# seungjunlee96/lightning-generative-models

Measured on AMD Instinct MI355X. Metric: training images/sec (DDPM UNet 32x32, bs=128), higher is better.
Workload: dtype f32

## Files before the change

### lightning-generative-models_amd/csrc/linattn_fused.hip

```cpp
#include <type_traits>

#include "lgm_common.h"

int lgm_wgrad_reduce_launch(const float* ws, long slab, float* gw, long n_w, float* gb, long n_b, int splits, float beta,
                            hipStream_t s);

namespace {

constexpr int DH = 32;
constexpr int HEADS = 4;
constexpr int HID = HEADS * DH;
constexpr int C = 64;
constexpr int LD = 36;
constexpr int TP = 128;
constexpr int XLD = 80;
constexpr int WLD = 100;

struct FArgs {
  const float* qkv;  long pitch;
  const float* gout; long gout_pitch;
  const float* ctx; const float* gctx; const float* kmax; const float* ksum; const float* rvec;
  const float* xn;   long xn_pitch;
  const float* wt;
  float* gxn;        long gxn_pitch;
  float* slabs;
  int n, tiles, items, per;
  float scale;
};

__device__ __forceinline__ void load16(const float* p, float (&v)[16]) {
#pragma unroll
  for (int q = 0; q < 4; ++q) {
    const f32x4 t = *reinterpret_cast<const f32x4*>(p + 4 * q);
    v[4 * q] = t[0]; v[4 * q + 1] = t[1]; v[4 * q + 2] = t[2]; v[4 * q + 3] = t[3];
  }
}

__global__ __launch_bounds__(256, 1) void linattn_bwd_fused_kernel(const FArgs p) {
  extern __shared__ __align__(16) float sm[];
  float* Qs = sm;
  float* Ks = Qs + TP * LD;
  float* Vs = Ks + TP * LD;
  float* Gs = Vs + TP * LD;
  float* Cs = Gs + TP * LD;
  float* GCs = Cs + DH * LD;
  float* GCt = GCs + DH * LD;
  float* rr = GCt + DH * LD;
  float* Ws = rr + DH;
  float* Xs = Ws + C * WLD;
  const int tid = threadIdx.x;
  const int lane = tid & 63, wid = tid >> 6;
  const int lr = lane & 31, lh = lane >> 5;
  const int l16 = lane & 15, lq = lane >> 4;
  const int c4 = (tid & 7) * 4, prow = tid >> 3;
  const int srow = 32 * wid + (lane >> 1), spart = (lane & 1) * 16;
  const int it0 = blockIdx.x * p.per, it1 = min(p.items, it0 + p.per);
  if (it0 >= it1) return;

  int w_src[6], w_dst[6];
#pragma unroll
  for (int u = 0; u < 6; ++u) {
    const int e = tid + 256 * u;
    const int c = e / 24, rem = e - 24 * c;
    const int part = rem >> 3, j = rem & 7;
    w_src[u] = c * (3 * HID) + part * HID + 4 * j;
    w_dst[u] = c * WLD + part * DH + 4 * j;
  }

  f32x4 q4[4], k4[4], v4[4], g4[4], km4, ks4, cx4, gc4, w4[6];
  float rr1 = 0.f;
  auto issue = [&](int it, int h) {
    const int b = it / p.tiles, i0 = (it % p.tiles) * TP;
    const int rows = min(TP, p.n - i0);
    const long bh = (long)b * HEADS + h;
#pragma unroll
    for (int u = 0; u < 4; ++u) {
      const int r = prow + 32 * u;
      const long row = (long)b * p.n + i0 + (r < rows ? r : 0);
      const float* qp = p.qkv + row * p.pitch + h * DH + c4;
      q4[u] = *reinterpret_cast<const f32x4*>(qp);
      k4[u] = *reinterpret_cast<const f32x4*>(qp + HID);
      v4[u] = *reinterpret_cast<const f32x4*>(qp + 2 * HID);
      g4[u] = *reinterpret_cast<const f32x4*>(p.gout + row * p.gout_pitch + h * DH + c4);
    }
    km4 = *reinterpret_cast<const f32x4*>(p.kmax + bh * DH + c4);
    ks4 = *reinterpret_cast<const f32x4*>(p.ksum + bh * DH + c4);
    cx4 = *reinterpret_cast<const f32x4*>(p.ctx + bh * DH * DH + tid * 4);
    gc4 = *reinterpret_cast<const f32x4*>(p.gctx + bh * DH * DH + tid * 4);
    if (tid < DH) rr1 = p.rvec[bh * DH + tid];
#pragma unroll
    for (int u = 0; u < 6; ++u) w4[u] = *reinterpret_cast<const f32x4*>(p.wt + w_src[u] + h * DH);
  };

  f32x4 dacc[HEADS][6];
#pragma unroll
  for (int h = 0; h < HEADS; ++h)
#pragma unroll
    for (int t = 0; t < 6; ++t) dacc[h][t] = f32x4{0.f, 0.f, 0.f, 0.f};
  const f32x4 zero4 = {0.f, 0.f, 0.f, 0.f};

  issue(it0, 0);
  for (int it = it0; it < it1; ++it) {
    const int b = it / p.tiles, i0 = (it % p.tiles) * TP;
    const int rows = min(TP, p.n - i0);
    f32x16 acc[2];
#pragma unroll
    for (int a = 0; a < 2; ++a)
#pragma unroll
      for (int r = 0; r < 16; ++r) acc[a][r] = 0.f;
    {
#pragma unroll
      for (int u = 0; u < 4; ++u) {
        const int r = prow + 32 * u;
        const long row = (long)b * p.n + i0 + (r < rows ? r : 0);
#pragma unroll
        for (int hf = 0; hf < 2; ++hf) {
          f32x4 xv = *reinterpret_cast<const f32x4*>(p.xn + row * p.xn_pitch + hf * 32 + c4);
          if (r >= rows) xv = zero4;
          *reinterpret_cast<f32x4*>(Xs + r * XLD + hf * 32 + c4) = xv;
        }
      }
    }
    auto head = [&](auto hc) {
      constexpr int h = decltype(hc)::value;
#pragma unroll
      for (int u = 0; u < 4; ++u) {
        const int r = prow + 32 * u;
        const bool live = r < rows;
        f32x4 kv;
#pragma unroll
        for (int k = 0; k < 4; ++k) kv[k] = __expf(k4[u][k] - km4[k]) * (1.f / ks4[k]);
        *reinterpret_cast<f32x4*>(Qs + r * LD + c4) = live ? q4[u] : zero4;
        *reinterpret_cast<f32x4*>(Ks + r * LD + c4) = live ? kv : zero4;
        *reinterpret_cast<f32x4*>(Vs + r * LD + c4) = live ? v4[u] : zero4;
        *reinterpret_cast<f32x4*>(Gs + r * LD + c4) = live ? g4[u] : zero4;
      }
      {
        const int d = tid >> 3, e0 = (tid & 7) * 4;
        *reinterpret_cast<f32x4*>(Cs + d * LD + e0) = cx4;
        *reinterpret_cast<f32x4*>(GCs + d * LD + e0) = gc4;
#pragma unroll
        for (int k = 0; k < 4; ++k) GCt[(e0 + k) * LD + d] = gc4[k];
      }
      if (tid < DH) rr[tid] = rr1;
#pragma unroll
      for (int u = 0; u < 6; ++u) *reinterpret_cast<f32x4*>(Ws + w_dst[u]) = w4[u];
      __syncthreads();
      if (h + 1 < HEADS) issue(it, h + 1);
      else if (it + 1 < it1) issue(it + 1, 0);

      float sv[16];
      {
        load16(Qs + srow * LD + spart, sv);
        float mx = sv[0];
#pragma unroll
        for (int k = 1; k < 16; ++k) mx = fmaxf(mx, sv[k]);
        mx = fmaxf(mx, __shfl_xor(mx, 1, 64));
        float sum = 0.f;
#pragma unroll
        for (int k = 0; k < 16; ++k) {
          sv[k] = __expf(sv[k] - mx);
          sum += sv[k];
        }
        sum += __shfl_xor(sum, 1, 64);
        const float inv = 1.f / sum;
#pragma unroll
        for (int k = 0; k < 16; ++k) sv[k] *= inv;
      }
      f32x16 a1, a2, a3;
#pragma unroll
      for (int r = 0; r < 16; ++r) a1[r] = a2[r] = a3[r] = 0.f;
      {
        float ca[16], ga[16], ta[16], gb[16], vb[16], kb[16];
        load16(Cs + lr * LD + 16 * lh, ca);
        load16(GCs + lr * LD + 16 * lh, ga);
        load16(GCt + lr * LD + 16 * lh, ta);
        load16(Gs + (32 * wid + lr) * LD + 16 * lh, gb);
        load16(Vs + (32 * wid + lr) * LD + 16 * lh, vb);
        load16(Ks + (32 * wid + lr) * LD + 16 * lh, kb);
#pragma unroll
        for (int s = 0; s < 16; ++s) {
          a1 = __builtin_amdgcn_mfma_f32_32x32x2f32(ca[s], gb[s], a1, 0, 0, 0);
          a2 = __builtin_amdgcn_mfma_f32_32x32x2f32(ga[s], vb[s], a2, 0, 0, 0);
          a3 = __builtin_amdgcn_mfma_f32_32x32x2f32(ta[s], kb[s], a3, 0, 0, 0);
        }
      }
      lgm_wave_lds_sync();
      {
        float* gp = Gs + (32 * wid + lr) * LD + 4 * lh;
        float* vp = Vs + (32 * wid + lr) * LD + 4 * lh;
#pragma unroll
        for (int g = 0; g < 4; ++g) {
          *reinterpret_cast<f32x4*>(gp + 8 * g) = f32x4{a1[4 * g], a1[4 * g + 1], a1[4 * g + 2], a1[4 * g + 3]};
          *reinterpret_cast<f32x4*>(vp + 8 * g) = f32x4{a2[4 * g], a2[4 * g + 1], a2[4 * g + 2], a2[4 * g + 3]};
        }
      }
      lgm_wave_lds_sync();
      {
        float g1[16], t2[16], kk[16], rv[16], dot = 0.f;
        load16(Gs + srow * LD + spart, g1);
        load16(Vs + srow * LD + spart, t2);
        load16(Ks + srow * LD + spart, kk);
        load16(rr + spart, rv);
#pragma unroll
        for (int k = 0; k < 16; ++k) {
          g1[k] *= p.scale;
          dot += sv[k] * g1[k];
        }
        dot += __shfl_xor(dot, 1, 64);
#pragma unroll
        for (int q = 0; q < 4; ++q) {
          f32x4 oq, ok;
#pragma unroll
          for (int k = 0; k < 4; ++k) {
            oq[k] = sv[4 * q + k] * (g1[4 * q + k] - dot);
            ok[k] = kk[4 * q + k] * (t2[4 * q + k] - rv[4 * q + k]);
          }
          *reinterpret_cast<f32x4*>(Qs + srow * LD + spart + 4 * q) = oq;
          *reinterpret_cast<f32x4*>(Ks + srow * LD + spart + 4 * q) = ok;
        }
      }
      lgm_wave_lds_sync();
      {
        float* vp = Vs + (32 * wid + lr) * LD + 4 * lh;
#pragma unroll
        for (int g = 0; g < 4; ++g)
          *reinterpret_cast<f32x4*>(vp + 8 * g) = f32x4{a3[4 * g], a3[4 * g + 1], a3[4 * g + 2], a3[4 * g + 3]};
      }
      lgm_wave_lds_sync();
#pragma unroll
      for (int part = 0; part < 3; ++part) {
        float xb[16], w0[16], w1[16];
        load16((part == 0 ? Qs : part == 1 ? Ks : Vs) + (32 * wid + lr) * LD + 16 * lh, xb);
        load16(Ws + lr * WLD + part * DH + 16 * lh, w0);
        load16(Ws + (32 + lr) * WLD + part * DH + 16 * lh, w1);
#pragma unroll
        for (int s = 0; s < 16; ++s) {
          acc[0] = __builtin_amdgcn_mfma_f32_32x32x2f32(w0[s], xb[s], acc[0], 0, 0, 0);
          acc[1] = __builtin_amdgcn_mfma_f32_32x32x2f32(w1[s], xb[s], acc[1], 0, 0, 0);
        }
      }
      __syncthreads();
      {
        const float* xb = Xs + lq * XLD + 16 * wid + l16;
#pragma unroll 4
        for (int s = 0; s < TP / 4; ++s) {
          const float bv = xb[4 * s * XLD];
#pragma unroll
          for (int part = 0; part < 3; ++part) {
            const float* X = (part == 0 ? Qs : part == 1 ? Ks : Vs) + (4 * s + lq) * LD + l16;
            dacc[h][2 * part] = __builtin_amdgcn_mfma_f32_16x16x4f32(X[0], bv, dacc[h][2 * part], 0, 0, 0);
            dacc[h][2 * part + 1] = __builtin_amdgcn_mfma_f32_16x16x4f32(X[16], bv, dacc[h][2 * part + 1], 0, 0, 0);
          }
        }
        __syncthreads();
      }
    };
    head(std::integral_constant<int, 0>{});
    head(std::integral_constant<int, 1>{});
    head(std::integral_constant<int, 2>{});
    head(std::integral_constant<int, 3>{});
    if (32 * wid + lr < rows) {
      float* o = p.gxn + ((long)b * p.n + i0 + 32 * wid + lr) * p.gxn_pitch + 4 * lh;
#pragma unroll
      for (int a = 0; a < 2; ++a)
#pragma unroll
        for (int g = 0; g < 4; ++g)
          *reinterpret_cast<f32x4*>(o + 32 * a + 8 * g) = f32x4{acc[a][4 * g], acc[a][4 * g + 1], acc[a][4 * g + 2], acc[a][4 * g + 3]};
    }
  }
  {
    float* sl = p.slabs + (long)blockIdx.x * (3 * HID * C);
#pragma unroll
    for (int h = 0; h < HEADS; ++h)
#pragma unroll
      for (int t = 0; t < 6; ++t)
#pragma unroll
        for (int r = 0; r < 4; ++r) {
          const int wrow = (t >> 1) * HID + h * DH + (t & 1) * 16 + 4 * lq + r;
          sl[(long)wrow * C + 16 * wid + l16] = dacc[h][t][r];
        }
  }
}

constexpr size_t kSmem = ((size_t)4 * TP * LD + 3 * DH * LD + DH + C * WLD + TP * XLD) * sizeof(float);

int plan_blocks(int B, int n, int* tiles, int* items, int* per) {
  *tiles = lgm_cdiv(n, TP);
  *items = B * *tiles;
  const int nb = *items < 256 ? *items : 256;
  *per = lgm_cdiv(*items, nb);
  return lgm_cdiv(*items, *per);
}

}

extern "C" int64_t lgm_linattn_bwd_fused_supported(int heads, int dim_head, int Cin) {
  return heads == HEADS && dim_head == DH && Cin == C ? 1 : 0;
}

extern "C" int64_t lgm_linattn_bwd_fused_slabs(int B, int n, int Cin) {
  if (Cin != C) return 0;
  int tiles, items, per;
  const int blocks = plan_blocks(B, n, &tiles, &items, &per);
  return (int64_t)blocks * 3 * HID * C * (int64_t)sizeof(float);
}

int lgm_linattn_bwd_fused_launch(const float* qkv, long pitch, const float* gout, long gout_pitch, const float* ctx,
                                 const float* gctx, const float* kmax, const float* ksum, const float* rvec,
                                 const float* xn, long xn_pitch, const float* wt, int B, int n, float scale,
                                 float* gxn, long gxn_pitch, float* slabs, int* blocks_out, hipStream_t s) {
  FArgs a;
  a.qkv = qkv; a.pitch = pitch; a.gout = gout; a.gout_pitch = gout_pitch;
  a.ctx = ctx; a.gctx = gctx; a.kmax = kmax; a.ksum = ksum; a.rvec = rvec;
  a.xn = xn; a.xn_pitch = xn_pitch; a.wt = wt; a.gxn = gxn; a.gxn_pitch = gxn_pitch;
  a.slabs = slabs; a.n = n; a.scale = scale;
  const int blocks = plan_blocks(B, n, &a.tiles, &a.items, &a.per);
  *blocks_out = blocks;
  lgm_note_kernel(LGM_KNAME("linattn_bwd_fused_kernel"));
  static bool attr = false;
  if (!attr) {
    (void)hipFuncSetAttribute(reinterpret_cast<const void*>(linattn_bwd_fused_kernel),
                              hipFuncAttributeMaxDynamicSharedMemorySize, (int)kSmem);
    attr = true;
  }
  hipLaunchKernelGGL(linattn_bwd_fused_kernel, dim3(blocks), dim3(256), kSmem, s, a);
  LGM_LAUNCH_CHECK();
  return LGM_OK;
}

namespace {

constexpr int OTP = 128;
constexpr int ALD = 132;

struct OArgs {
  const float* qkv;  long pitch;
  const float* ctx;
  const float* wout; const float* bout; const float* g;
  const float* x;    long x_pitch;
  float* ao;         long ao_pitch;
  float* o2;         long o2_pitch;
  float* y;          long y_pitch;
  int n, tiles, items, per;
  float scale;
};

template <int NC>
__global__ __launch_bounds__(256, NC == 2 ? 3 : 1) void linattn_out_fused_kernel(const OArgs p) {
  constexpr int CO = 32 * NC;
  extern __shared__ __align__(16) float sm[];
  float* Ws = sm;
  float* Ct = Ws + CO * ALD;
  const int tid = threadIdx.x;
  const int lane = tid & 63, wid = tid >> 6;
  const int lr = lane & 31, lh = lane >> 5;
  const int it0 = blockIdx.x * p.per, it1 = min(p.items, it0 + p.per);
  if (it0 >= it1) return;
  const float sqrtc = sqrtf((float)CO);

  f32x4 qn[4];
  auto issue_q = [&](int it, int h) {
    const int b = it / p.tiles, i0 = (it % p.tiles) * OTP;
    const int pix = min(i0 + 32 * wid + lr, p.n - 1);
    const float* qp = p.qkv + ((long)b * p.n + pix) * p.pitch + h * DH + 16 * lh;
#pragma unroll
    for (int j = 0; j < 4; ++j) qn[j] = *reinterpret_cast<const f32x4*>(qp + 4 * j);
  };
  issue_q(it0, 0);
#pragma unroll
  for (int u = 0; u < NC * 4; ++u) {
    const int e = tid + 256 * u;
    const int c = e >> 5, k4 = (e & 31) * 4;
    *reinterpret_cast<f32x4*>(Ws + c * ALD + k4) = *reinterpret_cast<const f32x4*>(p.wout + (long)c * HID + k4);
  }
  int b_staged = -1;
  for (int it = it0; it < it1; ++it) {
    const int b = it / p.tiles, i0 = (it % p.tiles) * OTP;
    const int pix = i0 + 32 * wid + lr;
    const bool live = pix < p.n;
    const long row = (long)b * p.n + min(pix, p.n - 1);
    if (b != b_staged) {
      __syncthreads();
#pragma unroll
      for (int u = 0; u < 4; ++u) {
        const int e = (tid + 256 * u) * 4;
        const int h = e >> 10, d = (e >> 5) & 31, e0 = e & 31;
        const f32x4 cv = *reinterpret_cast<const f32x4*>(p.ctx + (long)b * HEADS * DH * DH + e);
#pragma unroll
        for (int k = 0; k < 4; ++k) Ct[h * (DH * LD) + (e0 + k) * LD + d] = cv[k];
      }
      __syncthreads();
      b_staged = b;
    }
    f32x4 xres[NC <= 4 ? NC * 4 : 1];
    if constexpr (NC <= 4) {
#pragma unroll
      for (int a = 0; a < NC; ++a)
#pragma unroll
        for (int g = 0; g < 4; ++g)
          xres[a * 4 + g] = *reinterpret_cast<const f32x4*>(p.x + row * p.x_pitch + a * 32 + 8 * g + 4 * lh);
    }
    f32x16 acc[NC];
#pragma unroll
    for (int a = 0; a < NC; ++a)
#pragma unroll
      for (int r = 0; r < 16; ++r) acc[a][r] = 0.f;
#pragma unroll
    for (int h = 0; h < HEADS; ++h) {
      float qs[16];
#pragma unroll
      for (int j = 0; j < 4; ++j) {
        qs[4 * j] = qn[j][0]; qs[4 * j + 1] = qn[j][1]; qs[4 * j + 2] = qn[j][2]; qs[4 * j + 3] = qn[j][3];
      }
      if (h + 1 < HEADS) issue_q(it, h + 1);
      else if (it + 1 < it1) issue_q(it + 1, 0);
      float mx = qs[0];
#pragma unroll
      for (int k = 1; k < 16; ++k) mx = fmaxf(mx, qs[k]);
      mx = fmaxf(mx, __shfl_xor(mx, 32, 64));
      float sum = 0.f;
#pragma unroll
      for (int k = 0; k < 16; ++k) {
        qs[k] = __expf(qs[k] - mx);
        sum += qs[k];
      }
      sum += __shfl_xor(sum, 32, 64);
      const float inv = p.scale / sum;
      float ca[16];
      load16(Ct + h * (DH * LD) + lr * LD + 16 * lh, ca);
      f32x16 o;
#pragma unroll
      for (int r = 0; r < 16; ++r) o[r] = 0.f;
#pragma unroll
      for (int s = 0; s < 16; ++s) o = __builtin_amdgcn_mfma_f32_32x32x2f32(ca[s], qs[s] * inv, o, 0, 0, 0);
      if (live) {
#pragma unroll
        for (int g = 0; g < 4; ++g)
          *reinterpret_cast<f32x4*>(p.ao + row * p.ao_pitch + h * DH + 8 * g + 4 * lh) =
              f32x4{o[4 * g], o[4 * g + 1], o[4 * g + 2], o[4 * g + 3]};
      }
#pragma unroll
      for (int a = 0; a < NC; ++a) {
        const float* wp = Ws + (a * 32 + lr) * ALD + h * DH + 4 * lh;
#pragma unroll
        for (int g = 0; g < 4; ++g) {
          const f32x4 wv = *reinterpret_cast<const f32x4*>(wp + 8 * g);
#pragma unroll
          for (int j = 0; j < 4; ++j) acc[a] = __builtin_amdgcn_mfma_f32_32x32x2f32(wv[j], o[4 * g + j], acc[a], 0, 0, 0);
        }
      }
    }
    float ss = 0.f;
#pragma unroll
    for (int a = 0; a < NC; ++a)
#pragma unroll
      for (int g = 0; g < 4; ++g) {
        const f32x4 bv = *reinterpret_cast<const f32x4*>(p.bout + a * 32 + 8 * g + 4 * lh);
#pragma unroll
        for (int k = 0; k < 4; ++k) {
          acc[a][4 * g + k] += bv[k];
          ss += acc[a][4 * g + k] * acc[a][4 * g + k];
        }
      }
    ss += __shfl_xor(ss, 32, 64);
    const float rinv = sqrtc / fmaxf(sqrtf(ss), 1e-12f);
    if (live) {
#pragma unroll
      for (int a = 0; a < NC; ++a)
#pragma unroll
        for (int g = 0; g < 4; ++g) {
          const int c = a * 32 + 8 * g + 4 * lh;
          const f32x4 v = {acc[a][4 * g], acc[a][4 * g + 1], acc[a][4 * g + 2], acc[a][4 * g + 3]};
          const f32x4 gv = *reinterpret_cast<const f32x4*>(p.g + c);
          f32x4 xv;
          if constexpr (NC <= 4) xv = xres[a * 4 + g];
          else xv = *reinterpret_cast<const f32x4*>(p.x + row * p.x_pitch + c);
          *reinterpret_cast<f32x4*>(p.o2 + row * p.o2_pitch + c) = v;
          *reinterpret_cast<f32x4*>(p.y + row * p.y_pitch + c) = v * gv * rinv + xv;
        }
    }
  }
}

template <int NC>
int launch_out(const OArgs& a, int blocks, hipStream_t s) {
  const size_t smem = ((size_t)32 * NC * ALD + HEADS * DH * LD) * sizeof(float);
  static bool attr = false;
  if (!attr) {
    (void)hipFuncSetAttribute(reinterpret_cast<const void*>(linattn_out_fused_kernel<NC>),
                              hipFuncAttributeMaxDynamicSharedMemorySize, (int)smem);
    attr = true;
  }
  hipLaunchKernelGGL(linattn_out_fused_kernel<NC>, dim3(blocks), dim3(256), smem, s, a);
  LGM_LAUNCH_CHECK();
  return LGM_OK;
}

}

extern "C" int64_t lgm_linattn_fwd_fused_supported(int heads, int dim_head, int Cout) {
  if (heads != HEADS || dim_head != DH) return 0;
  return Cout == 64 || Cout == 128 ? 2 : Cout == 256 ? 1 : 0;
}

int lgm_linattn_out_fused_launch(const float* qkv, long pitch, const float* ctx, const float* wout, const float* bout,
                                 const float* g, const float* x, long x_pitch, float* ao, long ao_pitch, float* o2,
                                 long o2_pitch, float* y, long y_pitch, int B, int n, int Cout, float scale, hipStream_t s) {
  OArgs a;
  a.qkv = qkv; a.pitch = pitch; a.ctx = ctx; a.wout = wout; a.bout = bout; a.g = g; a.x = x; a.x_pitch = x_pitch;
  a.ao = ao; a.ao_pitch = ao_pitch; a.o2 = o2; a.o2_pitch = o2_pitch; a.y = y; a.y_pitch = y_pitch;
  a.n = n; a.scale = scale;
  a.tiles = lgm_cdiv(n, OTP);
  a.items = B * a.tiles;
  const int slots = Cout == 64 ? 768 : 256;
  const int nb = a.items < slots ? a.items : slots;
  a.per = lgm_cdiv(a.items, nb);
  const int blocks = lgm_cdiv(a.items, a.per);
  lgm_note_kernel(Cout == 64 ? LGM_KNAME("linattn_out_fused_kernel<2>") : Cout == 128 ? LGM_KNAME("linattn_out_fused_kernel<4>")
                                                                             : LGM_KNAME("linattn_out_fused_kernel<8>"));
  if (Cout == 64) return launch_out<2>(a, blocks, s);
  if (Cout == 128) return launch_out<4>(a, blocks, s);
  return launch_out<8>(a, blocks, s);
}

namespace {

struct QArgs {
  const float* x;  long x_pitch;
  const float* g;
  const float* w;
  float* xn;       long xn_pitch;
  float* qkv;      long q_pitch;
  long P;
  int items, per;
};

template <int NCI>
__global__ __launch_bounds__(256, NCI == 2 ? 3 : NCI == 4 ? 2 : 1) void rms_qkv_fused_kernel(const QArgs p) {
  constexpr int CI = 32 * NCI;
  constexpr int WL = CI + 4;
  extern __shared__ __align__(16) float sm[];
  float* Ws = sm;
  const int tid = threadIdx.x;
  const int lane = tid & 63, wid = tid >> 6;
  const int lr = lane & 31, lh = lane >> 5;
  int blk, slice;
  {
    const int nblk = (int)gridDim.x / 3, bid = (int)blockIdx.x;
    if (nblk % 8 == 0) {
      const int xcd = bid & 7, slot = bid >> 3;
      blk = (slot / 3) * 8 + xcd;
      slice = slot % 3;
    } else {
      blk = bid / 3;
      slice = bid % 3;
    }
  }
  const int it0 = blk * p.per, it1 = min(p.items, it0 + p.per);
  if (it0 >= it1) return;
  const float sqrtc = sqrtf((float)CI);
  f32x4 xr[NCI * 4];
  auto issue_x = [&](int it) {
    const long pix = (long)it * 128 + 32 * wid + lr;
    const long row = pix < p.P ? pix : p.P - 1;
#pragma unroll
    for (int a = 0; a < NCI; ++a)
#pragma unroll
      for (int g = 0; g < 4; ++g)
        xr[a * 4 + g] = *reinterpret_cast<const f32x4*>(p.x + row * p.x_pitch + a * 32 + 8 * g + 4 * lh);
  };
  issue_x(it0);
#pragma unroll
  for (int u = 0; u < NCI * 4; ++u) {
    const int e = tid + 256 * u;
    const int r = e / (CI / 4), c4 = (e % (CI / 4)) * 4;
    *reinterpret_cast<f32x4*>(Ws + r * WL + c4) = *reinterpret_cast<const f32x4*>(p.w + (long)(slice * 128 + r) * CI + c4);
  }
  __syncthreads();
  for (int it = it0; it < it1; ++it) {
    const long pix = (long)it * 128 + 32 * wid + lr;
    const bool live = pix < p.P;
    const long row = live ? pix : p.P - 1;
    f32x4 xn[NCI * 4];
    float ss = 0.f;
#pragma unroll
    for (int k = 0; k < NCI * 4; ++k) {
      xn[k] = xr[k];
      ss += xn[k][0] * xn[k][0] + xn[k][1] * xn[k][1] + xn[k][2] * xn[k][2] + xn[k][3] * xn[k][3];
    }
    if (NCI <= 4 && it + 1 < it1) issue_x(it + 1);
    ss += __shfl_xor(ss, 32, 64);
    const float inv = sqrtc / fmaxf(sqrtf(ss), 1e-12f);
#pragma unroll
    for (int a = 0; a < NCI; ++a)
#pragma unroll
      for (int g = 0; g < 4; ++g) {
        const f32x4 gv = *reinterpret_cast<const f32x4*>(p.g + a * 32 + 8 * g + 4 * lh);
        xn[a * 4 + g] = xn[a * 4 + g] * gv * inv;
        if (slice == 0 && live)
          *reinterpret_cast<f32x4*>(p.xn + row * p.xn_pitch + a * 32 + 8 * g + 4 * lh) = xn[a * 4 + g];
      }
#pragma unroll 1
    for (int t = 0; t < 4; ++t) {
      f32x16 acc;
#pragma unroll
      for (int r = 0; r < 16; ++r) acc[r] = 0.f;
      const float* wp = Ws + (t * 32 + lr) * WL + 4 * lh;
#pragma unroll
      for (int a = 0; a < NCI; ++a)
#pragma unroll
        for (int g = 0; g < 4; ++g) {
          const f32x4 wv = *reinterpret_cast<const f32x4*>(wp + a * 32 + 8 * g);
#pragma unroll
          for (int j = 0; j < 4; ++j) acc = __builtin_amdgcn_mfma_f32_32x32x2f32(wv[j], xn[a * 4 + g][j], acc, 0, 0, 0);
        }
      if (live) {
        float* o = p.qkv + row * p.q_pitch + slice * 128 + t * 32 + 4 * lh;
#pragma unroll
        for (int g = 0; g < 4; ++g)
          *reinterpret_cast<f32x4*>(o + 8 * g) = f32x4{acc[4 * g], acc[4 * g + 1], acc[4 * g + 2], acc[4 * g + 3]};
      }
    }
    if (NCI > 4 && it + 1 < it1) issue_x(it + 1);
  }
}

template <int NCI>
int launch_qkv(const QArgs& a, int blocks, hipStream_t s) {
  const size_t smem = (size_t)128 * (32 * NCI + 4) * sizeof(float);
  static bool attr = false;
  if (!attr) {
    (void)hipFuncSetAttribute(reinterpret_cast<const void*>(rms_qkv_fused_kernel<NCI>),
                              hipFuncAttributeMaxDynamicSharedMemorySize, (int)smem);
    attr = true;
  }
  hipLaunchKernelGGL(rms_qkv_fused_kernel<NCI>, dim3(blocks * 3), dim3(256), smem, s, a);
  LGM_LAUNCH_CHECK();
  return LGM_OK;
}

}

extern "C" int64_t lgm_rms_qkv_fused_supported(int C, int N) {
  if (N != 3 * HID) return 0;
  return C == 64 ? 2 : C == 128 || C == 256 ? 1 : 0;
}

extern "C" int lgm_rms_qkv_fused(const float* x, int64_t x_pitch, const float* g, const float* w, int C, int N,
                                 int64_t npix, float* xn, int64_t xn_pitch, float* qkv, int64_t qkv_pitch, void* stream) {
  LGM_REQUIRE(lgm_rms_qkv_fused_supported(C, N), "rms_qkv_fused: C=%d N=%d unsupported", C, N);
  LGM_REQUIRE(x && g && w && xn && qkv && npix > 0, "rms_qkv_fused: null pointer / empty");
  LGM_REQUIRE(x_pitch % 4 == 0 && xn_pitch % 4 == 0 && qkv_pitch % 4 == 0 && lgm_aligned16(x) && lgm_aligned16(g) &&
                  lgm_aligned16(w) && lgm_aligned16(xn) && lgm_aligned16(qkv),
              "rms_qkv_fused: 16-byte aligned operands required");
  QArgs a;
  a.x = x; a.x_pitch = x_pitch; a.g = g; a.w = w; a.xn = xn; a.xn_pitch = xn_pitch; a.qkv = qkv; a.q_pitch = qkv_pitch;
  a.P = npix;
  a.items = lgm_cdiv(npix, 128);
  const int slots = C == 64 ? 256 : C == 128 ? 170 : 85;
  const int nb = a.items < slots ? a.items : slots;
  a.per = lgm_cdiv(a.items, nb);
  const int blocks = lgm_cdiv(a.items, a.per);
  lgm_note_kernel(C == 64 ? LGM_KNAME("rms_qkv_fused_kernel<2>") : C == 128 ? LGM_KNAME("rms_qkv_fused_kernel<4>") : LGM_KNAME("rms_qkv_fused_kernel<8>"));
  hipStream_t s = (hipStream_t)stream;
  if (C == 64) return launch_qkv<2>(a, blocks, s);
  if (C == 128) return launch_qkv<4>(a, blocks, s);
  return launch_qkv<8>(a, blocks, s);
}
```

Measured before the change: 13220.

## Split linear-attention backward kernel across 512 threads with two wave halves

```diff
diff --git a/lightning-generative-models_amd/csrc/linattn_fused.hip b/lightning-generative-models_amd/csrc/linattn_fused.hip
--- a/lightning-generative-models_amd/csrc/linattn_fused.hip
+++ b/lightning-generative-models_amd/csrc/linattn_fused.hip
@@ -36,7 +36,7 @@
   }
 }
 
-__global__ __launch_bounds__(256, 1) void linattn_bwd_fused_kernel(const FArgs p) {
+__global__ __launch_bounds__(512, 2) void linattn_bwd_fused_kernel(const FArgs p) {
   extern __shared__ __align__(16) float sm[];
   float* Qs = sm;
   float* Ks = Qs + TP * LD;
@@ -49,33 +49,27 @@
   float* Ws = rr + DH;
   float* Xs = Ws + C * WLD;
   const int tid = threadIdx.x;
-  const int lane = tid & 63, wid = tid >> 6;
+  const int lane = tid & 63, wid = __builtin_amdgcn_readfirstlane(tid >> 6);
+  const int rg = wid & 3, half = wid >> 2;
   const int lr = lane & 31, lh = lane >> 5;
   const int l16 = lane & 15, lq = lane >> 4;
   const int c4 = (tid & 7) * 4, prow = tid >> 3;
-  const int srow = 32 * wid + (lane >> 1), spart = (lane & 1) * 16;
+  const int srow = 32 * rg + (lane >> 1), spart = (lane & 1) * 16;
   const int it0 = blockIdx.x * p.per, it1 = min(p.items, it0 + p.per);
   if (it0 >= it1) return;
 
-  int w_src[6], w_dst[6];
-#pragma unroll
-  for (int u = 0; u < 6; ++u) {
-    const int e = tid + 256 * u;
-    const int c = e / 24, rem = e - 24 * c;
-    const int part = rem >> 3, j = rem & 7;
-    w_src[u] = c * (3 * HID) + part * HID + 4 * j;
-    w_dst[u] = c * WLD + part * DH + 4 * j;
-  }
-
-  f32x4 q4[4], k4[4], v4[4], g4[4], km4, ks4, cx4, gc4, w4[6];
+  const int w_src = prow * (3 * HID) + c4, w_dst = prow * WLD + c4;
+
+  f32x4 q4[2], k4[2], v4[2], g4[2], km4, ks4, cg4, w4[3];
   float rr1 = 0.f;
+  const float* cgsrc = half == 0 ? p.ctx : p.gctx;
   auto issue = [&](int it, int h) {
     const int b = it / p.tiles, i0 = (it % p.tiles) * TP;
     const int rows = min(TP, p.n - i0);
     const long bh = (long)b * HEADS + h;
 #pragma unroll
-    for (int u = 0; u < 4; ++u) {
-      const int r = prow + 32 * u;
+    for (int u = 0; u < 2; ++u) {
+      const int r = prow + 64 * u;
       const long row = (long)b * p.n + i0 + (r < rows ? r : 0);
       const float* qp = p.qkv + row * p.pitch + h * DH + c4;
       q4[u] = *reinterpret_cast<const f32x4*>(qp);
@@ -85,33 +79,32 @@
     }
     km4 = *reinterpret_cast<const f32x4*>(p.kmax + bh * DH + c4);
     ks4 = *reinterpret_cast<const f32x4*>(p.ksum + bh * DH + c4);
-    cx4 = *reinterpret_cast<const f32x4*>(p.ctx + bh * DH * DH + tid * 4);
-    gc4 = *reinterpret_cast<const f32x4*>(p.gctx + bh * DH * DH + tid * 4);
+    cg4 = *reinterpret_cast<const f32x4*>(cgsrc + bh * DH * DH + (tid & 255) * 4);
     if (tid < DH) rr1 = p.rvec[bh * DH + tid];
-#pragma unroll
-    for (int u = 0; u < 6; ++u) w4[u] = *reinterpret_cast<const f32x4*>(p.wt + w_src[u] + h * DH);
   };
-
-  f32x4 dacc[HEADS][6];
+  auto issue_w = [&](int h) {
+#pragma unroll
+    for (int u = 0; u < 3; ++u) w4[u] = *reinterpret_cast<const f32x4*>(p.wt + w_src + u * HID + h * DH);
+  };
+
+  f32x4 dacc[HEADS][3];
 #pragma unroll
   for (int h = 0; h < HEADS; ++h)
 #pragma unroll
-    for (int t = 0; t < 6; ++t) dacc[h][t] = f32x4{0.f, 0.f, 0.f, 0.f};
+    for (int t = 0; t < 3; ++t) dacc[h][t] = f32x4{0.f, 0.f, 0.f, 0.f};
   const f32x4 zero4 = {0.f, 0.f, 0.f, 0.f};
-
   issue(it0, 0);
+  issue_w(0);
   for (int it = it0; it < it1; ++it) {
     const int b = it / p.tiles, i0 = (it % p.tiles) * TP;
     const int rows = min(TP, p.n - i0);
-    f32x16 acc[2];
-#pragma unroll
-    for (int a = 0; a < 2; ++a)
-#pragma unroll
-      for (int r = 0; r < 16; ++r) acc[a][r] = 0.f;
+    f32x16 acc;
+#pragma unroll
+    for (int r = 0; r < 16; ++r) acc[r] = 0.f;
     {
 #pragma unroll
-      for (int u = 0; u < 4; ++u) {
-        const int r = prow + 32 * u;
+      for (int u = 0; u < 2; ++u) {
+        const int r = prow + 64 * u;
         const long row = (long)b * p.n + i0 + (r < rows ? r : 0);
 #pragma unroll
         for (int hf = 0; hf < 2; ++hf) {
@@ -124,8 +117,8 @@
     auto head = [&](auto hc) {
       constexpr int h = decltype(hc)::value;
 #pragma unroll
-      for (int u = 0; u < 4; ++u) {
-        const int r = prow + 32 * u;
+      for (int u = 0; u < 2; ++u) {
+        const int r = prow + 64 * u;
         const bool live = r < rows;
         f32x4 kv;
 #pragma unroll
@@ -136,123 +129,145 @@
         *reinterpret_cast<f32x4*>(Gs + r * LD + c4) = live ? g4[u] : zero4;
       }
       {
-        const int d = tid >> 3, e0 = (tid & 7) * 4;
-        *reinterpret_cast<f32x4*>(Cs + d * LD + e0) = cx4;
-        *reinterpret_cast<f32x4*>(GCs + d * LD + e0) = gc4;
-#pragma unroll
-        for (int k = 0; k < 4; ++k) GCt[(e0 + k) * LD + d] = gc4[k];
+        const int d = (tid & 255) >> 3, e0 = (tid & 7) * 4;
+        if (half == 0) {
+          *reinterpret_cast<f32x4*>(Cs + d * LD + e0) = cg4;
+        } else {
+          *reinterpret_cast<f32x4*>(GCs + d * LD + e0) = cg4;
+#pragma unroll
+          for (int k = 0; k < 4; ++k) GCt[(e0 + k) * LD + d] = cg4[k];
+        }
       }
       if (tid < DH) rr[tid] = rr1;
 #pragma unroll
-      for (int u = 0; u < 6; ++u) *reinterpret_cast<f32x4*>(Ws + w_dst[u]) = w4[u];
+      for (int u = 0; u < 3; ++u) *reinterpret_cast<f32x4*>(Ws + w_dst + u * DH) = w4[u];
       __syncthreads();
       if (h + 1 < HEADS) issue(it, h + 1);
       else if (it + 1 < it1) issue(it + 1, 0);
 
-      float sv[16];
-      {
-        load16(Qs + srow * LD + spart, sv);
-        float mx = sv[0];
-#pragma unroll
-        for (int k = 1; k < 16; ++k) mx = fmaxf(mx, sv[k]);
-        mx = fmaxf(mx, __shfl_xor(mx, 1, 64));
-        float sum = 0.f;
-#pragma unroll
-        for (int k = 0; k < 16; ++k) {
-          sv[k] = __expf(sv[k] - mx);
-          sum += sv[k];
-        }
-        sum += __shfl_xor(sum, 1, 64);
-        const float inv = 1.f / sum;
-#pragma unroll
-        for (int k = 0; k < 16; ++k) sv[k] *= inv;
-      }
-      f32x16 a1, a2, a3;
-#pragma unroll
-      for (int r = 0; r < 16; ++r) a1[r] = a2[r] = a3[r] = 0.f;
-      {
-        float ca[16], ga[16], ta[16], gb[16], vb[16], kb[16];
-        load16(Cs + lr * LD + 16 * lh, ca);
-        load16(GCs + lr * LD + 16 * lh, ga);
-        load16(GCt + lr * LD + 16 * lh, ta);
-        load16(Gs + (32 * wid + lr) * LD + 16 * lh, gb);
-        load16(Vs + (32 * wid + lr) * LD + 16 * lh, vb);
-        load16(Ks + (32 * wid + lr) * LD + 16 * lh, kb);
-#pragma unroll
-        for (int s = 0; s < 16; ++s) {
-          a1 = __builtin_amdgcn_mfma_f32_32x32x2f32(ca[s], gb[s], a1, 0, 0, 0);
-          a2 = __builtin_amdgcn_mfma_f32_32x32x2f32(ga[s], vb[s], a2, 0, 0, 0);
-          a3 = __builtin_amdgcn_mfma_f32_32x32x2f32(ta[s], kb[s], a3, 0, 0, 0);
-        }
-      }
-      lgm_wave_lds_sync();
-      {
-        float* gp = Gs + (32 * wid + lr) * LD + 4 * lh;
-        float* vp = Vs + (32 * wid + lr) * LD + 4 * lh;
-#pragma unroll
-        for (int g = 0; g < 4; ++g) {
+      float* gp = Gs + (32 * rg + lr) * LD + 4 * lh;
+      float* vp = Vs + (32 * rg + lr) * LD + 4 * lh;
+      if (half == 0) {
+        float sv[16];
+        {
+          load16(Qs + srow * LD + spart, sv);
+          float mx = sv[0];
+#pragma unroll
+          for (int k = 1; k < 16; ++k) mx = fmaxf(mx, sv[k]);
+          mx = fmaxf(mx, __shfl_xor(mx, 1, 64));
+          float sum = 0.f;
+#pragma unroll
+          for (int k = 0; k < 16; ++k) {
+            sv[k] = __expf(sv[k] - mx);
+            sum += sv[k];
+          }
+          sum += __shfl_xor(sum, 1, 64);
+          const float inv = 1.f / sum;
+#pragma unroll
+          for (int k = 0; k < 16; ++k) sv[k] *= inv;
+        }
+        f32x16 a1;
+#pragma unroll
+        for (int r = 0; r < 16; ++r) a1[r] = 0.f;
+        {
+          float ca[16], gb[16];
+          load16(Cs + lr * LD + 16 * lh, ca);
+          load16(Gs + (32 * rg + lr) * LD + 16 * lh, gb);
+#pragma unroll
+          for (int s = 0; s < 16; ++s) a1 = __builtin_amdgcn_mfma_f32_32x32x2f32(ca[s], gb[s], a1, 0, 0, 0);
+        }
+        lgm_wave_lds_sync();
+#pragma unroll
+        for (int g = 0; g < 4; ++g)
           *reinterpret_cast<f32x4*>(gp + 8 * g) = f32x4{a1[4 * g], a1[4 * g + 1], a1[4 * g + 2], a1[4 * g + 3]};
+        lgm_wave_lds_sync();
+        {
+          float g1[16], dot = 0.f;
+          load16(Gs + srow * LD + spart, g1);
+#pragma unroll
+          for (int k = 0; k < 16; ++k) {
+            g1[k] *= p.scale;
+            dot += sv[k] * g1[k];
+          }
+          dot += __shfl_xor(dot, 1, 64);
+#pragma unroll
+          for (int q = 0; q < 4; ++q) {
+            f32x4 oq;
+#pragma unroll
+            for (int k = 0; k < 4; ++k) oq[k] = sv[4 * q + k] * (g1[4 * q + k] - dot);
+            *reinterpret_cast<f32x4*>(Qs + srow * LD + spart + 4 * q) = oq;
+          }
+        }
+      } else {
+        f32x16 a2, a3;
+#pragma unroll
+        for (int r = 0; r < 16; ++r) a2[r] = a3[r] = 0.f;
+        {
+          float ga[16], vb[16];
+          load16(GCs + lr * LD + 16 * lh, ga);
+          load16(Vs + (32 * rg + lr) * LD + 16 * lh, vb);
+#pragma unroll
+          for (int s = 0; s < 16; ++s) a2 = __builtin_amdgcn_mfma_f32_32x32x2f32(ga[s], vb[s], a2, 0, 0, 0);
+        }
+        {
+          float ta[16], kb[16];
+          load16(GCt + lr * LD + 16 * lh, ta);
+          load16(Ks + (32 * rg + lr) * LD + 16 * lh, kb);
+#pragma unroll
+          for (int s = 0; s < 16; ++s) a3 = __builtin_amdgcn_mfma_f32_32x32x2f32(ta[s], kb[s], a3, 0, 0, 0);
+        }
+        lgm_wave_lds_sync();
+#pragma unroll
+        for (int g = 0; g < 4; ++g)
           *reinterpret_cast<f32x4*>(vp + 8 * g) = f32x4{a2[4 * g], a2[4 * g + 1], a2[4 * g + 2], a2[4 * g + 3]};
-        }
-      }
-      lgm_wave_lds_sync();
-      {
-        float g1[16], t2[16], kk[16], rv[16], dot = 0.f;
-        load16(Gs + srow * LD + spart, g1);
-        load16(Vs + srow * LD + spart, t2);
-        load16(Ks + srow * LD + spart, kk);
-        load16(rr + spart, rv);
-#pragma unroll
-        for (int k = 0; k < 16; ++k) {
-          g1[k] *= p.scale;
-          dot += sv[k] * g1[k];
-        }
-        dot += __shfl_xor(dot, 1, 64);
-#pragma unroll
-        for (int q = 0; q < 4; ++q) {
-          f32x4 oq, ok;
-#pragma unroll
-          for (int k = 0; k < 4; ++k) {
-            oq[k] = sv[4 * q + k] * (g1[4 * q + k] - dot);
-            ok[k] = kk[4 * q + k] * (t2[4 * q + k] - rv[4 * q + k]);
+        lgm_wave_lds_sync();
+        {
+          float t2[16], kk[16], rv[16];
+          load16(Vs + srow * LD + spart, t2);
+          load16(Ks + srow * LD + spart, kk);
+          load16(rr + spart, rv);
+#pragma unroll
+          for (int q = 0; q < 4; ++q) {
+            f32x4 ok;
+#pragma unroll
+            for (int k = 0; k < 4; ++k) ok[k] = kk[4 * q + k] * (t2[4 * q + k] - rv[4 * q + k]);
+            *reinterpret_cast<f32x4*>(Ks + srow * LD + spart + 4 * q) = ok;
           }
-          *reinterpret_cast<f32x4*>(Qs + srow * LD + spart + 4 * q) = oq;
-          *reinterpret_cast<f32x4*>(Ks + srow * LD + spart + 4 * q) = ok;
-        }
-      }
-      lgm_wave_lds_sync();
-      {
-        float* vp = Vs + (32 * wid + lr) * LD + 4 * lh;
+        }
+        lgm_wave_lds_sync();
 #pragma unroll
         for (int g = 0; g < 4; ++g)
           *reinterpret_cast<f32x4*>(vp + 8 * g) = f32x4{a3[4 * g], a3[4 * g + 1], a3[4 * g + 2], a3[4 * g + 3]};
       }
-      lgm_wave_lds_sync();
+      __syncthreads();
 #pragma unroll
       for (int part = 0; part < 3; ++part) {
-        float xb[16], w0[16], w1[16];
-        load16((part == 0 ? Qs : part == 1 ? Ks : Vs) + (32 * wid + lr) * LD + 16 * lh, xb);
-        load16(Ws + lr * WLD + part * DH + 16 * lh, w0);
-        load16(Ws + (32 + lr) * WLD + part * DH + 16 * lh, w1);
-#pragma unroll
-        for (int s = 0; s < 16; ++s) {
-          acc[0] = __builtin_amdgcn_mfma_f32_32x32x2f32(w0[s], xb[s], acc[0], 0, 0, 0);
-          acc[1] = __builtin_amdgcn_mfma_f32_32x32x2f32(w1[s], xb[s], acc[1], 0, 0, 0);
-        }
-      }
-      __syncthreads();
+        float xb[16], w0[16];
+        load16((part == 0 ? Qs : part == 1 ? Ks : Vs) + (32 * rg + lr) * LD + 16 * lh, xb);
+        load16(Ws + (32 * half + lr) * WLD + part * DH + 16 * lh, w0);
+#pragma unroll
+        for (int s = 0; s < 16; ++s) acc = __builtin_amdgcn_mfma_f32_32x32x2f32(w0[s], xb[s], acc, 0, 0, 0);
+      }
+      if (h + 1 < HEADS) issue_w(h + 1);
+      else if (it + 1 < it1) issue_w(0);
       {
-        const float* xb = Xs + lq * XLD + 16 * wid + l16;
+        const float* xb = Xs + lq * XLD + 16 * rg + l16;
+        auto tiles = [&](auto hv) {
+          constexpr int hf = decltype(hv)::value;
 #pragma unroll 4
-        for (int s = 0; s < TP / 4; ++s) {
-          const float bv = xb[4 * s * XLD];
-#pragma unroll
-          for (int part = 0; part < 3; ++part) {
-            const float* X = (part == 0 ? Qs : part == 1 ? Ks : Vs) + (4 * s + lq) * LD + l16;
-            dacc[h][2 * part] = __builtin_amdgcn_mfma_f32_16x16x4f32(X[0], bv, dacc[h][2 * part], 0, 0, 0);
-            dacc[h][2 * part + 1] = __builtin_amdgcn_mfma_f32_16x16x4f32(X[16], bv, dacc[h][2 * part + 1], 0, 0, 0);
+          for (int s = 0; s < TP / 4; ++s) {
+            const float bv = xb[4 * s * XLD];
+            const float* X = Qs + (4 * s + lq) * LD + l16;
+#pragma unroll
+            for (int j = 0; j < 3; ++j) {
+              constexpr int t0 = 3 * hf;
+              const int t = t0 + j;
+              dacc[h][j] = __builtin_amdgcn_mfma_f32_16x16x4f32(X[(t >> 1) * (TP * LD) + 16 * (t & 1)], bv, dacc[h][j], 0, 0, 0);
+            }
           }
-        }
+        };
+        if (half == 0) tiles(std::integral_constant<int, 0>{});
+        else tiles(std::integral_constant<int, 1>{});
         __syncthreads();
       }
     };
@@ -260,25 +275,24 @@
     head(std::integral_constant<int, 1>{});
     head(std::integral_constant<int, 2>{});
     head(std::integral_constant<int, 3>{});
-    if (32 * wid + lr < rows) {
-      float* o = p.gxn + ((long)b * p.n + i0 + 32 * wid + lr) * p.gxn_pitch + 4 * lh;
-#pragma unroll
-      for (int a = 0; a < 2; ++a)
-#pragma unroll
-        for (int g = 0; g < 4; ++g)
-          *reinterpret_cast<f32x4*>(o + 32 * a + 8 * g) = f32x4{acc[a][4 * g], acc[a][4 * g + 1], acc[a][4 * g + 2], acc[a][4 * g + 3]};
+    if (32 * rg + lr < rows) {
+      float* o = p.gxn + ((long)b * p.n + i0 + 32 * rg) * p.gxn_pitch + 32 * half + (lr * (int)p.gxn_pitch + 4 * lh);
+#pragma unroll
+      for (int g = 0; g < 4; ++g)
+        *reinterpret_cast<f32x4*>(o + 8 * g) = f32x4{acc[4 * g], acc[4 * g + 1], acc[4 * g + 2], acc[4 * g + 3]};
     }
   }
   {
-    float* sl = p.slabs + (long)blockIdx.x * (3 * HID * C);
+    float* sl = p.slabs + (long)blockIdx.x * (3 * HID * C) + 16 * rg + 4 * lq * C + l16;
 #pragma unroll
     for (int h = 0; h < HEADS; ++h)
 #pragma unroll
-      for (int t = 0; t < 6; ++t)
+      for (int j = 0; j < 3; ++j)
 #pragma unroll
         for (int r = 0; r < 4; ++r) {
-          const int wrow = (t >> 1) * HID + h * DH + (t & 1) * 16 + 4 * lq + r;
-          sl[(long)wrow * C + 16 * wid + l16] = dacc[h][t][r];
+          const int t = 3 * half + j;
+          const int wrow = (t >> 1) * HID + h * DH + (t & 1) * 16 + r;
+          sl[wrow * C] = dacc[h][j][r];
         }
   }
 }
@@ -324,7 +338,7 @@
                               hipFuncAttributeMaxDynamicSharedMemorySize, (int)kSmem);
     attr = true;
   }
-  hipLaunchKernelGGL(linattn_bwd_fused_kernel, dim3(blocks), dim3(256), kSmem, s, a);
+  hipLaunchKernelGGL(linattn_bwd_fused_kernel, dim3(blocks), dim3(512), kSmem, s, a);
   LGM_LAUNCH_CHECK();
   return LGM_OK;
 }
```

New measurement: 13340, median of 6. No clear change (+0.9%).
